# MycroftAI/mycroft-precise

Hardware: NVIDIA H100
Metric: stream-updates/s (16 kHz int16 PCM, 1024-sample chunk -> decoded confidence + trigger) (higher is better)
Workload: dtype f32

## Files before the change

### include/precise_b200.h

```cpp
#ifndef PRECISE_B200_H
#define PRECISE_B200_H

#include <stdint.h>

#ifdef __cplusplus
extern "C" {
#endif

#define PB_ABI_VERSION 2
#define PB_MAX_THRESHOLDS 8
#define PB_MAX_MODELS 8

typedef enum pb_status {
    PB_OK = 0,
    PB_ERR_INVALID = -1,
    PB_ERR_UNSUPPORTED = -2,
    PB_ERR_CUDA = -3,
    PB_ERR_STATE = -4,
    PB_ERR_EOF = -5
} pb_status;

enum { PB_VEC_MELS = 1, PB_VEC_MFCCS = 2, PB_VEC_SPEECHPY_MFCCS = 3  };
enum { PB_ACT_LINEAR = 0, PB_ACT_TANH = 1 };
enum { PB_RACT_HARD_SIGMOID = 0, PB_RACT_SIGMOID = 1 };
// ... 207 lines not shown

int pb_host_alloc(void** out, uint64_t bytes);
int pb_host_free(void* p);

int pb_profile_enable(pb_handle* h, int on);
int pb_profile_reset(pb_handle* h);
int pb_profile_read(pb_handle* h, double ms[4], uint64_t launches[4]);

int pb_get_filterbank(const pb_handle* h, double* h_out);
int64_t pb_get_cdf(const pb_handle* h, double* h_out, int64_t capacity, int32_t* min_out, int32_t* max_out);
int pb_set_cdf(pb_handle* h, const double* h_cd, int64_t len);

int pb_debug_force_generic(pb_handle* h, int on);
int pb_debug_gru_mode(pb_handle* h, int mode);
int pb_debug_k1_mode(pb_handle* h, int mode);
int pb_debug_pool_tiles(pb_handle* h, int warp_only);
int pb_debug_corpus_pool_rows(pb_handle* h, int64_t rows);
int pb_debug_corpus_pool_scan(pb_handle* h, int32_t nm, int32_t groups_fast);
int pb_debug_corpus_pairs_batch(pb_handle* h, int64_t windows);
int pb_debug_tc_dft_power(const int16_t* x512, double* power257);
int pb_debug_mma_dft_power(const int16_t* x512, double* power257);
int pb_debug_tc_mfcc_frame(const pb_config* cfg, const int16_t* x512, float* out);
int pb_debug_tc3_mfcc_frame(const pb_config* cfg, const int16_t* x512, float* out, double* power257);

const char* pb_last_error(void);
int pb_abi_version(void);
const char* pb_build_info(void);

#ifdef __cplusplus
}
// ... 3 lines not shown
```

### mycroft_precise_b200/core.py

```python
import ctypes as C
import os

import numpy as np

from .params import ListenerParams

_HERE = os.path.dirname(os.path.abspath(__file__))
PB_MAX_THRESHOLDS = 8
PB_MAX_MODELS = 8
PB_ABI_VERSION = 2
CORPUS_SCHEDULES = {'listener': 0, 'simulate': 1}
FRONT_END_FIELDS = ('sample_rate', 'window_samples', 'hop_samples', 'n_fft', 'n_filt', 'n_mfcc', 'n_features',
                    'use_delta', 'vectorizer')


class PBError(RuntimeError):
    pass


class pb_config(C.Structure):
    _fields_ = [
        ('abi_version', C.c_int32), ('device', C.c_int32), ('max_streams', C.c_int32),
        ('chunk_samples', C.c_int32),
        ('sample_rate', C.c_int32), ('window_samples', C.c_int32), ('hop_samples', C.c_int32),
# ... 78 lines not shown
    'pb_generate': (C.c_int, [_VP, _VP, _VP, _I64, _VP, _VP, _I64, _VP, _I64, _VP, _I64, _VP, _I64, _I64, _I32, _VP, _VP, _VP]),
    'pb_train_opts_default': (C.c_int, [C.POINTER(pb_train_opts)]),
    'pb_train': (C.c_int, [_VP, _VP, _I64, _VP, _VP, _I64, _VP, _VP, _I64, C.POINTER(pb_train_opts), _VP, _VP, _VP, _VP]),
    'pb_train_loss': (C.c_int, [_VP, _VP, _I64, _VP, _VP, _I64, _VP, _VP, _I64, C.c_float, C.c_float, _I32, _VP, _VP, _VP, _VP]),
    'pb_host_alloc': (C.c_int, [C.POINTER(_VP), C.c_uint64]),
    'pb_host_free': (C.c_int, [_VP]),
    'pb_profile_enable': (C.c_int, [_VP, C.c_int]),
    'pb_profile_reset': (C.c_int, [_VP]),
    'pb_profile_read': (C.c_int, [_VP, C.POINTER(C.c_double), C.POINTER(C.c_uint64)]),
    'pb_get_filterbank': (C.c_int, [_VP, _VP]),
    'pb_get_cdf': (_I64, [_VP, _VP, _I64, C.POINTER(_I32), C.POINTER(_I32)]),
    'pb_set_cdf': (C.c_int, [_VP, _VP, _I64]),
    'pb_debug_force_generic': (C.c_int, [_VP, C.c_int]),
    'pb_debug_gru_mode': (C.c_int, [_VP, C.c_int]),
    'pb_debug_k1_mode': (C.c_int, [_VP, C.c_int]),
    'pb_debug_pool_tiles': (C.c_int, [_VP, C.c_int]),
    'pb_debug_corpus_pool_rows': (C.c_int, [_VP, _I64]),
    'pb_debug_corpus_pool_scan': (C.c_int, [_VP, _I32, _I32]),
    'pb_debug_corpus_pairs_batch': (C.c_int, [_VP, _I64]),
    'pb_debug_tc_dft_power': (C.c_int, [_VP, _VP]),
    'pb_debug_mma_dft_power': (C.c_int, [_VP, _VP]),
    'pb_debug_tc_mfcc_frame': (C.c_int, [_VP, _VP, _VP]),
    'pb_debug_tc3_mfcc_frame': (C.c_int, [_VP, _VP, _VP, _VP]),
    'pb_last_error': (C.c_char_p, []),
    'pb_abi_version': (C.c_int, []),
    'pb_build_info': (C.c_char_p, []),
}

_lib = None

# ... 918 lines not shown
        cnt = C.c_uint64(0)
        vp = _np_ptr
        check(self.lib.pb_update_host(self._h, vp(pcm_np), vp(ids_np), n, vp(raw_np), vp(conf_np), vp(fired_np),
                                      C.cast(C.byref(cnt), C.c_void_p)))
        return int(cnt.value)

    def gru_mode(self, mode):
        check(self.lib.pb_debug_gru_mode(self._h, int(mode)))

    def force_generic(self, on=True):
        check(self.lib.pb_debug_force_generic(self._h, int(on)))

    def k1_mode(self, mode):
        check(self.lib.pb_debug_k1_mode(self._h, int(mode)))

    def profile(self, on=True):
        check(self.lib.pb_profile_enable(self._h, int(on)))
        check(self.lib.pb_profile_reset(self._h))

    def profile_read(self):
        ms = (C.c_double * 4)()
        ln = (C.c_uint64 * 4)()
        check(self.lib.pb_profile_read(self._h, ms, ln))
        return list(ms), list(ln)

    def filterbank(self) -> np.ndarray:
        fb = np.zeros((self.params.n_filt, self.params.n_fft // 2 + 1), dtype=np.float64)
        check(self.lib.pb_get_filterbank(self._h, fb.ctypes.data_as(C.c_void_p)))
        return fb

# ... 22 lines not shown
```

### mycroft_precise_b200/csrc/api.cu

```cuda
#include <cuda_runtime.h>
#include <math.h>
#include <stdarg.h>
#include <stdint.h>
#include <stdio.h>
#include <string.h>

#include <algorithm>
#include <map>
#include <cuda_fp16.h>
#include <limits>
#include <memory>
#include <mutex>
#include <new>
#include <string>
#include <utility>
#include <vector>

#include "../../include/precise_b200.h"
#include "gru_kernels.cuh"
#include "gru_bank.cuh"
#include "gru_wg.cuh"
#include "gru_wide.cuh"
#include "mfcc_kernels.cuh"
#include "mfcc_fast.cuh"
// ... 129 lines not shown
    int mm_parity = 0;
    bool fast_ok = false;
    int npl = 0, maxc = 0, nol = 0;
    DevArray<float4> d_ptab;
    DevArray<unsigned char> d_ctab;
    DevArray<float> d_dct_t;
    bool pipe_fixed = false;
    DevArray<int4> d_pm_off; DevArray<float4> d_pm_w; DevArray<uint4> d_pm_crow; DevArray<float4> d_pm_dct;
    std::vector<double> fb;
    DevArray<float> d_wrise, d_wfall, d_dct;
    DevArray<int> d_grid;
    DevArray<float2> d_tw_stage, d_tw_post, d_tw_any;
    DevArray<long long> d_n_samples;
    DevArray<int16_t> d_tail;
    DevArray<float> d_ring;
    std::vector<Network> models;
    bool routed = false;
    std::vector<uint8_t> route_mask;
    int64_t subs[PB_MAX_MODELS] = {};
    DevArray<uint8_t> d_route;
    DevArray<int2> d_route_list;
    DevArray<unsigned> d_route_count;
    cudaEvent_t route_ev = nullptr;
    bool history = false;
    int64_t hist_samples = 0;
    int hist_cap = 0;
    int hist_rows = 0;
    DevArray<int16_t> d_hist;
    DevArray<int> d_hist_row;
    DevArray<long long> d_hist_start;
// ... 52 lines not shown
    bool pool_warp_only = false;
    bool pool_trig_set = false;
    std::vector<StreamTrig> pool_trig_host;
    DevArray<TrigRec> d_pool_trig_rec;
    cudaStream_t pipe[HOST_PIPE] = {nullptr, nullptr, nullptr};
    cudaEvent_t pipe_ev[HOST_PIPE] = {nullptr, nullptr, nullptr};
    DevArray<int16_t> d_stage_pcm[HOST_PIPE];
    DevArray<int> d_stage_ids[HOST_PIPE];
    DevArray<float> d_stage_raw[HOST_PIPE];
    DevArray<double> d_stage_conf[HOST_PIPE];
    DevArray<uint8_t> d_stage_fired[HOST_PIPE];
    DevArray<unsigned long long> d_count;
    unsigned long long* h_count_pinned = nullptr;
    bool profiling = false;
    ProfSlot prof[N_PROFILE_SLOTS];

    pb_handle() = default;
    pb_handle(const pb_handle&) = delete;
    pb_handle& operator=(const pb_handle&) = delete;
    ~pb_handle() {
        if (h_count_pinned) cudaFreeHost(h_count_pinned);
        for (int i = 0; i < HOST_PIPE; ++i) {
            if (pipe[i]) cudaStreamDestroy(pipe[i]);
            if (pipe_ev[i]) cudaEventDestroy(pipe_ev[i]);
        }
        for (auto& p : prof)
            for (auto e : p.ev) cudaEventDestroy(e);
        if (route_ev) cudaEventDestroy(route_ev);
        if (corpus_ev) cudaEventDestroy(corpus_ev);
        if (pool_ev) cudaEventDestroy(pool_ev);
    }
};

struct MelHost {
    std::vector<int> grid;
    std::vector<float> wrise, wfall;
    std::vector<double> fb;
};

static int build_mel(const pb_config& c, int n_bins, MelHost& mel) {
    const int nb = n_bins, nf = c.n_filt;
    const double top = 1127.0 * log(1.0 + (double)c.sample_rate / 700.0);
    std::vector<int>& grid = mel.grid;
    std::vector<double>& fb = mel.fb;
    grid.assign(nf + 2, 0);
    long long shift = 0, prev = -1;
    if (c.vectorizer == PB_VEC_SPEECHPY_MFCCS) {
// ... 288 lines not shown
        std::vector<float4> pd((size_t)16 * NF / 4, make_float4(0.f, 0.f, 0.f, 0.f));
        for (int k = 0; k < h->n_out; ++k)
            for (int n = 0; n < NF; ++n) reinterpret_cast<float*>(pd.data())[(size_t)k * NF + n] = dct[(size_t)k * NF + n];
        CK(h->d_pm_off.upload(poff));
        CK(h->d_pm_w.upload(pw));
        CK(h->d_pm_crow.upload(crow));
        CK(h->d_pm_dct.upload(pd));
    }
    const size_t S = (size_t)c.max_streams;
    CK(h->d_n_samples.alloc(S));
    CK(h->d_tail.alloc(S * h->tail_cap));
    CK(h->d_ring.alloc(S * h->ring_rows * h->row_stride));
    CK(cudaMemset(h->d_n_samples.get(), 0, S * sizeof(long long)));
    CK(cudaMemset(h->d_tail.get(), 0, S * h->tail_cap * sizeof(int16_t)));
    CK(cudaMemset(h->d_ring.get(), 0, S * h->ring_rows * h->row_stride * sizeof(float)));
    CK(h->d_count.alloc(1));
    CK(cudaMemset(h->d_count.get(), 0, sizeof(unsigned long long)));
    CK(ensure_dyn_smem(mfcc_batch_kernel<int16_t, true>, (size_t)(h->k1_batch_smem)));
    CK(ensure_dyn_smem(mfcc_batch_kernel<int16_t, false>, (size_t)(h->k1_batch_smem)));
    CK(ensure_dyn_smem(mfcc_batch_kernel<float, true>, (size_t)(h->k1_batch_smem)));
    CK(ensure_dyn_smem(mfcc_batch_kernel<float, false>, (size_t)(h->k1_batch_smem)));
    CK(ensure_dyn_smem(mfcc_fast_batch_kernel, (size_t)(h->k1_fast_smem)));
    CK(ensure_dyn_smem(mfcc_fast_stream_kernel<false>, (size_t)(h->k1_fast_smem)));
    CK(ensure_dyn_smem(mfcc_fast_stream_kernel<true>, (size_t)(h->k1_fast_smem)));
    {
        auto kp = h->pipe_fixed ? mfcc_pipe_stream_kernel<K1P_FIX_NPL, K1P_FIX_MAXC, K1P_FIX_NF, K1P_FIX_NOUT> : mfcc_pipe_stream_kernel<0, 0, 0, 0>;
        CK(ensure_dyn_smem(kp, (size_t)(h->k1_pipe_smem)));
        CK(cudaFuncSetAttribute(kp, cudaFuncAttributePreferredSharedMemoryCarveout, (int)cudaSharedmemCarveoutMaxShared));
    }
    CK(ensure_dyn_smem(mfcc_stream_kernel<true>, (size_t)(h->k1_stream_smem)));
    CK(ensure_dyn_smem(mfcc_stream_kernel<false>, (size_t)(h->k1_stream_smem)));
    CK(ensure_dyn_smem(mfcc_stream_kernel<false, true>, (size_t)(h->k1_stream_smem)));
    CK(ensure_dyn_smem(mfcc_ragged_stream_kernel, (size_t)(h->k1_ragged_smem)));
    CK(ensure_dyn_smem(mfcc_fast_corpus_kernel, (size_t)(h->k1_fast_smem)));
    CK(ensure_dyn_smem(mfcc_corpus_kernel, (size_t)(h->k1_batch_smem)));

    Network net;
    net.cfg = c;
    build_cdf(net);
    CK(upload_network_state(net, S));
    h->models.push_back(std::move(net));
// ... 176 lines not shown
        CK(ensure_dyn_smem(gru_tiled_kernel<false>, tiled_smem));
    }
    net.w = std::move(w);
    return PB_OK;
}

PB_API int pb_load_weights(pb_handle* h, const float* kernel, const float* recurrent, const float* bias,
                    const float* dense_w, float dense_b) {
    if (!h || !kernel || !recurrent || !bias || !dense_w) return fail(PB_ERR_INVALID, "null argument");
    CK(cudaSetDevice(h->cfg.device));
    return load_weights(h->models[0], h->feat, kernel, recurrent, bias, dense_w, dense_b);
}

struct ProfScope {
    pb_handle* h; int slot; cudaStream_t s; int idx = -1;
    ProfScope(pb_handle* h_, int slot_, cudaStream_t s_) : h(h_), slot(slot_), s(s_) {
        if (!h->profiling) return;
        ProfSlot& p = h->prof[slot];
        if (p.used + 2 > (int)p.ev.size()) {
            if ((int)p.ev.size() >= 2 * PROFILE_POOL) {
                for (int i = 0; i + 1 < p.used; i += 2) {
                    cudaEventSynchronize(p.ev[i + 1]);
                    float ms = 0; cudaEventElapsedTime(&ms, p.ev[i], p.ev[i + 1]); p.ms += ms;
                }
                p.used = 0;
            } else {
                cudaEvent_t a, b; cudaEventCreate(&a); cudaEventCreate(&b); p.ev.push_back(a); p.ev.push_back(b);
            }
        }
        idx = p.used; p.used += 2; p.launches++;
        cudaEventRecord(p.ev[idx], s);
    }
    ~ProfScope() { if (idx >= 0) cudaEventRecord(h->prof[slot].ev[idx + 1], s); }
};

PB_API int pb_debug_gru_mode(pb_handle* h, int mode) {
    if (!h) return fail(PB_ERR_INVALID, "null handle");
    if (mode < 0 || mode > 2) return fail(PB_ERR_INVALID, "gru mode must be 0 (automatic), 1 (CUDA-core kernel) or 2 (tensor-core kernel)");
    h->models[0].gru_mode = mode;
    return PB_OK;
}

PB_API int pb_debug_k1_mode(pb_handle* h, int mode) {
    if (!h) return fail(PB_ERR_INVALID, "null handle");
    if (mode < 0 || mode > 6 || mode == 1) return fail(PB_ERR_INVALID, "k1 mode must be 0 (automatic), 2 (FFT kernel, lean set-up, not pipelined), 3 (FFT kernel, 64-bit set-up), 4 (tensor-core DFT stage 2), 5 (both DFT stages on the tensor cores) or 6 (5 with a shuffle epilogue)");
    if (mode != 0 && h->ragged) return fail(PB_ERR_STATE, "k1 modes 2-6 need 16-byte-aligned stream state, which a handle loses with its first pb_update_ragged");
    if (mode >= 4 && !h->mma_ok) return fail(PB_ERR_UNSUPPORTED, "the tensor-core MFCC tick needs n_fft = 512 = frame length, hop >= 512 (a multiple of 8), chunk >= hop (a multiple of 8), n_filt <= 32, MFCC vectorizer");
    if ((mode == 2 || mode == 3) && !h->fast_ok) return fail(PB_ERR_UNSUPPORTED, "k1 modes 2 and 3 need the aligned geometry of the fast MFCC kernels");
    h->k1_mode = mode;
    return PB_OK;
}

PB_API int pb_debug_tc_dft_power(const int16_t* x512, double* power257) {
    if (!x512 || !power257) return fail(PB_ERR_INVALID, "null argument");
// ... 65 lines not shown
}

PB_API int pb_debug_mma_dft_power(const int16_t* x512, double* power257) {
    if (!x512 || !power257) return fail(PB_ERR_INVALID, "null argument");
    mm_host_power(x512, power257);
    return PB_OK;
}

PB_API int pb_debug_force_generic(pb_handle* h, int on) { if (!h) return fail(PB_ERR_INVALID, "null handle"); h->force_generic = on != 0; return PB_OK; }

PB_API int pb_profile_enable(pb_handle* h, int on) { if (!h) return fail(PB_ERR_INVALID, "null handle"); h->profiling = on != 0; return PB_OK; }

PB_API int pb_profile_reset(pb_handle* h) {
    if (!h) return fail(PB_ERR_INVALID, "null handle");
    for (auto& p : h->prof) { p.used = 0; p.ms = 0; p.launches = 0; }
    return PB_OK;
}

PB_API int pb_profile_read(pb_handle* h, double ms[4], uint64_t launches[4]) {
    if (!h) return fail(PB_ERR_INVALID, "null handle");
    CK(cudaSetDevice(h->cfg.device));
    for (int s = 0; s < N_PROFILE_SLOTS; ++s) {
        ProfSlot& p = h->prof[s];
        for (int i = 0; i + 1 < p.used; i += 2) {
            CK(cudaEventSynchronize(p.ev[i + 1]));
            float t = 0; CK(cudaEventElapsedTime(&t, p.ev[i], p.ev[i + 1])); p.ms += t;
        }
        p.used = 0;
        if (ms) ms[s] = p.ms;
        if (launches) launches[s] = p.launches;
    }
    return PB_OK;
}

static MelTables mel_tables(const pb_handle* h) {
    MelTables t;
// ... 102 lines not shown
    const NetWeights& nw = *net.w;
    BankModelW& w = P.w[slot];
    w.bfrag = nw.bfrag16.get(); w.xfrag = nw.xfrag16.get(); w.bias = nw.mma_bias.get(); w.wd = nw.mma_wd.get(); w.bd = nw.bd;
    w.act = net.cfg.activation; w.ract = net.cfg.recurrent_activation;
    P.dp[slot] = decode_params(net);
    P.o[slot] = o;
}

template <int NM, bool RING, bool KERAS_ACT>
static int launch_bank_act(const BankParams& P, const K2In& in, int64_t n, cudaStream_t s) {
    constexpr size_t smem = (size_t)NM * BANK_MODEL_SMEM + (bank_stages(NM, RING) ? BANK_STAGE_SMEM : 0);
    const int per_cta = (MMA_THREADS / 32) * 16;
    const int grid = (int)((n + per_cta - 1) / per_cta);
    if constexpr (NM == 1) {
        if constexpr (smem > 48 * 1024) CK(ensure_dyn_smem(gru_wg_kernel<RING, KERAS_ACT>, smem));
        gru_wg_kernel<RING, KERAS_ACT><<<grid, MMA_THREADS, smem, s>>>(P, in, n);
    } else {
        if constexpr (smem > 48 * 1024) CK(ensure_dyn_smem(gru_bank_kernel<NM, RING, KERAS_ACT>, smem));
        gru_bank_kernel<NM, RING, KERAS_ACT><<<grid, MMA_THREADS, smem, s>>>(P, in, n);
    }
    CK(cudaGetLastError());
    return PB_OK;
}

template <int NM, bool RING>
static int launch_bank_nm(const BankParams& P, const K2In& in, int64_t n, cudaStream_t s) {
    if constexpr (NM == 1)
        if (P.w[0].act == PB_ACT_LINEAR && P.w[0].ract == PB_RACT_HARD_SIGMOID) return launch_bank_act<1, RING, true>(P, in, n, s);
    return launch_bank_act<NM, RING, false>(P, in, n, s);
}

// ... 109 lines not shown
    const int grid = (int)std::min<int64_t>((n + K1_STREAMS_PER_CTA - 1) / K1_STREAMS_PER_CTA, (int64_t)h->sm_count * 4);
    ProfScope ps(h, 0, s);
    for (int64_t off = 0; off < max_len; off += rg.sub) {
        rg.round_off = off;
        if (fast)
            mfcc_ragged_stream_kernel<<<gridf, K1F_THREADS, h->k1_ragged_smem, s>>>(d_pcm, rg, d_ids, (int)n, h->cfg.hop_samples, spw, scale,
                                                                                   mel_tables(h), fast_tables(h), st);
        else
            mfcc_stream_kernel<false, true><<<grid, K1_THREADS, h->k1_stream_smem, s>>>(d_pcm, d_ids, (int)n, 0, 0, h->cfg.hop_samples, h->used,
                                                                                       scale, mel_tables(h), st, rg);
        CK(cudaGetLastError());
    }
    return PB_OK;
}

static int launch_stream_mfcc(pb_handle* h, const int16_t* d_pcm, const int32_t* d_ids, int64_t n, cudaStream_t s) {
    if (h->ragged) return launch_ragged_mfcc(h, d_pcm, nullptr, h->cfg.chunk_samples, d_ids, n, s);
    const bool pairs = (h->cfg.chunk_samples % 2 == 0) && (h->cfg.hop_samples % 2 == 0) && (h->used % 2 == 0) &&
                       ((uintptr_t)d_pcm % 4 == 0);
    const int64_t tiles = (n + K1_STREAMS_PER_CTA - 1) / K1_STREAMS_PER_CTA;
    const int grid = (int)std::min<int64_t>(tiles, (int64_t)h->sm_count * 4);
    const float inv = 1.0f / 32768.0f, scale = inv * inv / (float)h->cfg.n_fft;
    const StreamState st = stream_state(h);
    ProfScope ps(h, 0, s);
    if (h->k1_mode >= 4 && h->mma_ok && (uintptr_t)d_pcm % 16 == 0 && !h->force_generic) {
        int rc = ensure_mma_tables(h);
        if (rc != PB_OK) return rc;
        MmTables t;
        t.b1 = h->d_mm_b1.get(); t.b2 = h->d_mm_b2.get(); t.tw = h->d_mm_tw.get();
        t.pscale = inv * inv / (float)h->cfg.n_fft * 1024.f;
        const int par = h->mm_parity;
        h->mm_parity ^= 1;
        MmRec* recs = h->d_mm_recs.get();
        unsigned int* counters = h->d_mm_counters.get();
        mfcc_mma_plan_kernel<<<(int)((n + MM_PLAN_THREADS - 1) / MM_PLAN_THREADS), MM_PLAN_THREADS, 0, s>>>(
            d_pcm, d_ids, (int)n, h->cfg.chunk_samples, h->cfg.hop_samples, st, recs, counters, par);
        const int64_t max_tiles = (n * std::max(1, h->max_new) + MM_FRAMES - 1) / MM_FRAMES;
        const int gm = (int)std::min<int64_t>((max_tiles + MM_WARPS - 1) / MM_WARPS, h->sm_count);
        if (h->k1_mode == 4)
            mfcc_mma_kernel<false, false><<<gm, MM_THREADS, sizeof(MmSmem), s>>>(t, mel_tables(h), recs, counters, par);
        else if (h->k1_mode == 5)
            mfcc_mma_kernel<true, false><<<gm, MM_THREADS, sizeof(MmSmem), s>>>(t, mel_tables(h), recs, counters, par);
        else
            mfcc_mma_kernel<true, true><<<gm, MM_THREADS, sizeof(MmSmem), s>>>(t, mel_tables(h), recs, counters, par);
    } else if (h->fast_ok && h->max_new <= 8 && h->cfg.chunk_samples % 8 == 0 && (uintptr_t)d_pcm % 16 == 0 && !h->force_generic) {
        const int64_t warps_total = (int64_t)h->sm_count * 4 * K1F_WARPS;
        const int spw = (int)std::max<int64_t>(1, std::min<int64_t>(K1F_STREAMS_PER_WARP, (n + warps_total - 1) / warps_total));
        const int64_t tilesf = (n + spw - 1) / spw;
        const int gridf = (int)std::min<int64_t>((tilesf + K1F_WARPS - 1) / K1F_WARPS, (int64_t)h->sm_count * 4);
        if (h->k1_mode == 0) {
            const int gridp = (int)std::min<int64_t>((tilesf + K1F_WARPS - 1) / K1F_WARPS, (int64_t)h->sm_count * K1P_CTAS_PER_SM);
            PipeMelTables pm;
            pm.poff = h->d_pm_off.get(); pm.pw = h->d_pm_w.get(); pm.crow = h->d_pm_crow.get(); pm.dct = h->d_pm_dct.get();
            auto kp = h->pipe_fixed ? mfcc_pipe_stream_kernel<K1P_FIX_NPL, K1P_FIX_MAXC, K1P_FIX_NF, K1P_FIX_NOUT> : mfcc_pipe_stream_kernel<0, 0, 0, 0>;
            kp<<<gridp, K1F_THREADS, h->k1_pipe_smem, s>>>(d_pcm, d_ids, (int)n, h->cfg.chunk_samples, h->cfg.hop_samples, spw, scale,
                                                           mel_tables(h), fast_tables(h), pm, st);
        } else if (h->k1_mode != 3)
            mfcc_fast_stream_kernel<true><<<gridf, K1F_THREADS, h->k1_fast_smem, s>>>(d_pcm, d_ids, (int)n, h->cfg.chunk_samples, h->cfg.hop_samples, spw, scale,
                                                                                      mel_tables(h), fast_tables(h), st);
        else
            mfcc_fast_stream_kernel<false><<<gridf, K1F_THREADS, h->k1_fast_smem, s>>>(d_pcm, d_ids, (int)n, h->cfg.chunk_samples, h->cfg.hop_samples, spw, scale,
                                                                                       mel_tables(h), fast_tables(h), st);
    } else if (h->max_new > 8) {
        const int sub = std::max(1, 6 * h->cfg.hop_samples);
        for (int off = 0; off < h->cfg.chunk_samples; off += sub)
            mfcc_stream_kernel<false><<<grid, K1_THREADS, h->k1_stream_smem, s>>>(d_pcm + off, d_ids, (int)n, std::min(sub, h->cfg.chunk_samples - off),
                                                                                    h->cfg.chunk_samples, h->cfg.hop_samples, h->used, scale, mel_tables(h), st, RaggedIn{});
    } else if (pairs)
        mfcc_stream_kernel<true><<<grid, K1_THREADS, h->k1_stream_smem, s>>>(d_pcm, d_ids, (int)n, h->cfg.chunk_samples, h->cfg.chunk_samples, h->cfg.hop_samples, h->used, scale, mel_tables(h), st, RaggedIn{});
    else
        mfcc_stream_kernel<false><<<grid, K1_THREADS, h->k1_stream_smem, s>>>(d_pcm, d_ids, (int)n, h->cfg.chunk_samples, h->cfg.chunk_samples, h->cfg.hop_samples, h->used, scale, mel_tables(h), st, RaggedIn{});
// ... 11 lines not shown
                          int64_t n, cudaStream_t s) {
    if (!h->history) return PB_OK;
    RaggedIn rg{};
    rg.offsets = reinterpret_cast<const long long*>(d_offsets);
    rg.max_len = max_len;
    rg.chunk = h->cfg.chunk_samples;
    rg.sub = (int)std::min<int64_t>(max_len, INT32_MAX);
    const int per = HIST_THREADS / 32;
    ProfScope ps(h, 3, s);
    history_append_kernel<<<(unsigned)((n + per - 1) / per), HIST_THREADS, 0, s>>>(d_pcm, rg, d_ids, (int)n, h->d_n_samples.get(),
                                                                                  hist_pool(h));
    CK(cudaGetLastError());
    return PB_OK;
}

static int tick_mfcc(pb_handle* h, const int16_t* d_pcm, const int32_t* d_ids, int64_t n, cudaStream_t s) {
    const int rc = append_history(h, d_pcm, nullptr, h->cfg.chunk_samples, d_ids, n, s);
    return rc != PB_OK ? rc : launch_stream_mfcc(h, d_pcm, d_ids, n, s);
}

PB_API int pb_update_vectors(pb_handle* h, const int16_t* d_pcm, const int32_t* d_ids, int64_t n, void* stream) {
    int rc = check_tick(h, d_pcm, n);
    if (rc != PB_OK || n == 0) return rc;
    CK(cudaSetDevice(h->cfg.device));
    return tick_mfcc(h, d_pcm, d_ids, n, (cudaStream_t)stream);
}

static K2In stream_k2in(const pb_handle* h, const int32_t* d_ids) {
    K2In in{};
    in.ring = h->d_ring.get(); in.n_samples = h->d_n_samples.get(); in.ids = d_ids;
    in.ring_rows = h->ring_rows; in.row_stride = h->row_stride; in.window = h->rel_window; in.hop = h->cfg.hop_samples;
    in.T = h->cfg.n_features; in.F_base = h->n_out; in.use_delta = h->cfg.use_delta;
    return in;
}

static int score_model0(pb_handle* h, const int32_t* d_ids, int64_t n, float* d_raw, double* d_conf, uint8_t* d_fired,
                        unsigned long long* d_count, cudaStream_t s) {
    const Network& net = h->models[0];
    K2Out o{};
    o.raw = d_raw; o.conf = d_conf; o.fired = d_fired; o.count = d_count; o.trig = net.trig.get();
    if (!h->routed && !net.trig_set) return launch_gru(h, net, stream_k2in(h, d_ids), true, n, o, s);
    TrigTick t{};
    t.ids = d_ids; t.n = n;
    int nt = 0;
    if (net.trig_set) defer_trigger(t, nt, net, 1u, o);
    ProfScope ps(h, 1, s);
    if (h->routed) {
        RouteOut r{};
        r.raw = d_raw; r.conf = d_conf; r.fired = d_fired; r.M = 1;
        route_kernel<<<(int)((n + 255) / 256), 256, 0, s>>>(h->d_route.get(), d_ids, n, r);
        CK(cudaGetLastError());
        if (h->subs[0] == 0) return PB_OK;
        o.route = h->d_route.get(); o.route_bit = 1;
        t.route = h->d_route.get();
    }
    const int rc = launch_gru_kernels(net, h->feat, stream_k2in(h, d_ids), true, n, o, s);
    return rc != PB_OK ? rc : launch_trigger(t, nt, s);
}

PB_API int pb_update(pb_handle* h, const int16_t* d_pcm, const int32_t* d_ids, int64_t n, float* d_raw, double* d_conf,
              uint8_t* d_fired, unsigned long long* d_count, void* stream) {
    int rc = check_tick(h, d_pcm, n);
    if (rc != PB_OK || n == 0) return rc;
    const Network& net = h->models[0];
    if (!net.w) return fail(PB_ERR_STATE, "pb_load_weights has not been called");
    if (!d_conf) return fail(PB_ERR_INVALID, "null d_conf");
    CK(cudaSetDevice(h->cfg.device));
    cudaStream_t s = (cudaStream_t)stream;
    rc = tick_mfcc(h, d_pcm, d_ids, n, s);
    if (rc != PB_OK) return rc;
    return score_model0(h, d_ids, n, d_raw, d_conf, d_fired, d_count, s);
}


static int check_front_end(const pb_handle* h, const pb_config& c) {
    if (c.abi_version != PB_ABI_VERSION) return fail(PB_ERR_INVALID, "abi_version %d != %d", c.abi_version, PB_ABI_VERSION);
#define PB_SAME_FRONT_END(f)                                                                                  \
    if (c.f != h->cfg.f)                                                                                      \
        return fail(PB_ERR_INVALID, "front-end field %s = %d differs from the handle's %d: the models of a bank share one MFCC front end", \
                    #f, (int)c.f, (int)h->cfg.f)
    PB_SAME_FRONT_END(sample_rate); PB_SAME_FRONT_END(window_samples); PB_SAME_FRONT_END(hop_samples); PB_SAME_FRONT_END(n_fft);
    PB_SAME_FRONT_END(n_filt); PB_SAME_FRONT_END(n_mfcc); PB_SAME_FRONT_END(n_features); PB_SAME_FRONT_END(use_delta);
    PB_SAME_FRONT_END(vectorizer); PB_SAME_FRONT_END(chunk_samples); PB_SAME_FRONT_END(device);
#undef PB_SAME_FRONT_END
    return PB_OK;
}
// ... 2490 lines not shown
```

### mycroft_precise_b200/csrc/gru_kernels.cuh

```cuda
#pragma once
#include <cuda_runtime.h>
#include <stdint.h>

namespace pb {

struct DecodeParams {
    const double* cd;
    int cd_len;
    int min_out, out_range;
    double center;
    double hot_threshold;
    int trigger_level;
    int trigger_reset;
    int legacy_f64;
};

struct K2Out {
    float* raw;
    float* logit;
    double* conf;
    uint8_t* fired;
    unsigned long long* count;
    int* trig;
    const uint8_t* route;
    unsigned route_bit;
};

struct K2In {
    const float* inputs;
    const float* ring;
    union {
        const long long* n_samples;
        const long long* starts;
    };
    const int* ids;
    int ring_rows, row_stride, window, hop;
    int T, F_base;
    int use_delta;
};

__device__ __forceinline__ const float* input_row(const K2In& in, long long i, int t) {
    return in.inputs + ((in.starts ? in.starts[i] : i * in.T) + t) * (long long)in.row_stride;
}

__device__ __forceinline__ float input_value(const K2In& in, long long i, int t, int f) {
    const float* row = input_row(in, i, t);
    if (!in.use_delta || f < in.F_base) return __ldg(row + f);
    const int fb = f - in.F_base;
    return t > 0 ? __ldg(row + fb) - __ldg(row + fb - in.row_stride) : 0.f;
}

__device__ __forceinline__ float hard_sigmoid(float x) { return fminf(fmaxf(fmaf(0.2f, x, 0.5f), 0.f), 1.f); }
__device__ __forceinline__ float sigmoid32(float x) { return 1.f / (1.f + expf(-x)); }
// ... 471 lines not shown
```

### mycroft_precise_b200/csrc/gru_wg.cuh

```cuda
#pragma once
#include <stdint.h>

#include "gru_bank.cuh"

namespace pb {

constexpr int WG_TILE_BYTES = 72 * 16 * 2;
__host__ __device__ constexpr int wg_b_offset(int k, int n) { return (n >> 3) * 256 + (k >> 3) * 128 + (n & 7) * 16 + (k & 7) * 2; }

__device__ __forceinline__ uint64_t wg_desc(const void* p) {
    const uint32_t a = (uint32_t)__cvta_generic_to_shared(p);
    return (uint64_t)((a & 0x3ffff) >> 4) | ((uint64_t)(128 >> 4) << 16) | ((uint64_t)(256 >> 4) << 32);
}

__device__ __forceinline__ void wg_fence() { asm volatile("wgmma.fence.sync.aligned;" ::: "memory"); }
__device__ __forceinline__ void wg_commit() { asm volatile("wgmma.commit_group.sync.aligned;" ::: "memory"); }
template <int N>
__device__ __forceinline__ void wg_wait() { asm volatile("wgmma.wait_group.sync.aligned %0;" :: "n"(N) : "memory"); }
__device__ __forceinline__ void wg_fence_smem() { asm volatile("fence.proxy.async.shared::cta;" ::: "memory"); }
template <int N>
__device__ __forceinline__ void wg_fence_regs(float* d) {
#pragma unroll
    for (int i = 0; i < N; ++i) asm volatile("" : "+f"(d[i]) :: "memory");
}
// ... 22 lines not shown
                 "{%0,%1,%2,%3,%4,%5,%6,%7,%8,%9,%10,%11,%12,%13,%14,%15,%16,%17,%18,%19,%20,%21,%22,%23,"
                 "%24,%25,%26,%27,%28,%29,%30,%31,%32,%33,%34,%35}, {%36,%37,%38,%39}, %40, p, 1, 1, 0;\n}\n"
                 : "+f"(d[0]), "+f"(d[1]), "+f"(d[2]), "+f"(d[3]), "+f"(d[4]), "+f"(d[5]), "+f"(d[6]), "+f"(d[7]),
                   "+f"(d[8]), "+f"(d[9]), "+f"(d[10]), "+f"(d[11]), "+f"(d[12]), "+f"(d[13]), "+f"(d[14]), "+f"(d[15]),
                   "+f"(d[16]), "+f"(d[17]), "+f"(d[18]), "+f"(d[19]), "+f"(d[20]), "+f"(d[21]), "+f"(d[22]), "+f"(d[23]),
                   "+f"(d[24]), "+f"(d[25]), "+f"(d[26]), "+f"(d[27]), "+f"(d[28]), "+f"(d[29]), "+f"(d[30]), "+f"(d[31]),
                   "+f"(d[32]), "+f"(d[33]), "+f"(d[34]), "+f"(d[35])
                 : "r"(a[0]), "r"(a[1]), "r"(a[2]), "r"(a[3]), "l"(desc), "r"(1));
}

template <bool RING, bool KERAS_ACT>
__global__ void __launch_bounds__(MMA_THREADS, 4)
gru_wg_kernel(const __grid_constant__ BankParams P, K2In in, long long n) {
    extern __shared__ __align__(16) unsigned char bank_smem[];
    const BankModelW& w = P.w[0];
    unsigned char* sW = bank_smem;
    float* sb = reinterpret_cast<float*>(bank_smem + BANK_FRAG_U4 * 16);
    for (int e = threadIdx.x; e < 3 * MMA_NT * 32; e += blockDim.x) {
        const int kt = e / (MMA_NT * 32), nt = (e / 32) % MMA_NT, lane = e & 31, col = 8 * nt + (lane >> 2), k = 2 * (lane & 3);
        const uint4 f = kt < 2 ? __ldg(w.bfrag + e) : __ldg(w.xfrag + e - 2 * MMA_NT * 32);
        unsigned char* hi = sW + (kt == 2 ? 0 : 2 + 2 * kt) * WG_TILE_BYTES;
        unsigned char* lo = hi + WG_TILE_BYTES;
        *reinterpret_cast<uint32_t*>(hi + wg_b_offset(k, col)) = f.x;
        *reinterpret_cast<uint32_t*>(hi + wg_b_offset(k + 8, col)) = f.y;
        *reinterpret_cast<uint32_t*>(lo + wg_b_offset(k, col)) = f.z;
        *reinterpret_cast<uint32_t*>(lo + wg_b_offset(k + 8, col)) = f.w;
    }
    for (int e = threadIdx.x; e < 72; e += blockDim.x) sb[e] = __ldg(w.bias + e);
    for (int e = threadIdx.x; e < 24; e += blockDim.x) sb[72 + e] = __ldg(w.wd + e);
    wg_fence_smem();
// ... 6 lines not shown
    int sid[2];
    bool ok[2];
#pragma unroll
    for (int hf = 0; hf < 2; ++hf) {
        idx[hf] = base + g + 8 * hf;
        ok[hf] = idx[hf] < n;
        sid[hf] = RING && ok[hf] ? (in.ids ? in.ids[idx[hf]] : (int)idx[hf]) : 0;
    }
    float* stage = reinterpret_cast<float*>(bank_smem + BANK_MODEL_SMEM) + warp * 2 * BANK_STAGE_BUF;
    const int cs = lane >> 1;
    const bool cok = STAGE && base + cs < n;
    RingCursor cur;
    cur.stride = 0;
    if (cok) {
        const int csid = in.ids ? in.ids[base + cs] : (int)(base + cs);
        const long long ns = in.n_samples[csid];
        cur.init(in, csid, ns >= in.window ? (ns - in.window) / in.hop + 1 : 0);
    }
    if (STAGE) {
        bank_stage(stage, cur, cok, cs, 0, in.T, in.ring, lane);
        cp_async_commit();
        bank_stage(stage + BANK_STAGE_BUF, cur, cok, cs, BANK_STAGE_STEPS, in.T, in.ring, lane);
        cp_async_commit();
    }
    const uint64_t dXh = wg_desc(sW), dXl = wg_desc(sW + WG_TILE_BYTES), dU0h = wg_desc(sW + 2 * WG_TILE_BYTES),
                   dU0l = wg_desc(sW + 3 * WG_TILE_BYTES), dU1h = wg_desc(sW + 4 * WG_TILE_BYTES), dU1l = wg_desc(sW + 5 * WG_TILE_BYTES);
    constexpr uint64_t C6 = (6 * 256) >> 4;
    const int ra = w.ract, ac = w.act;
    int chunk = 0, cr = 0;
    float h[3][4] = {};
// ... 104 lines not shown
    }
    if (STAGE) cp_async_wait<0>();
    const float* sWd = sb + 72;
#pragma unroll
    for (int hf = 0; hf < 2; ++hf) {
        float part = 0.f;
#pragma unroll
        for (int nt = 0; nt < 3; ++nt) {
            part = fmaf(h[nt][2 * hf], sWd[8 * nt + 2 * t], part);
            part = fmaf(h[nt][2 * hf + 1], sWd[8 * nt + 2 * t + 1], part);
        }
        part += __shfl_xor_sync(0xffffffffu, part, 1);
        part += __shfl_xor_sync(0xffffffffu, part, 2);
        epilogue(part + w.bd, t == 0 && ok[hf], idx[hf], sid[hf], P.dp[0], P.o[0]);
    }
}

}
```

### mycroft_precise_b200/csrc/mfcc_fast.cuh

```cuda
#pragma once
#include <cuda_runtime.h>
#include <stdint.h>
#include "fft512.cuh"
#include "mfcc_kernels.cuh"

namespace pb {

__device__ __forceinline__ uint32_t smem_u32(const void* p) { return (uint32_t)__cvta_generic_to_shared(p); }

__device__ __forceinline__ void mbar_init(unsigned long long* bar, uint32_t count) {
    asm volatile("mbarrier.init.shared::cta.b64 [%0], %1;" ::"r"(smem_u32(bar)), "r"(count) : "memory");
}
__device__ __forceinline__ void mbar_arrive(unsigned long long* bar) {
    asm volatile("mbarrier.arrive.shared::cta.b64 _, [%0];" ::"r"(smem_u32(bar)) : "memory");
}
__device__ __forceinline__ void mbar_expect_tx(unsigned long long* bar, uint32_t bytes) {
    asm volatile("mbarrier.arrive.expect_tx.shared::cta.b64 _, [%0], %1;" ::"r"(smem_u32(bar)), "r"(bytes) : "memory");
}
__device__ __forceinline__ void bulk_g2s(void* dst, const void* src, uint32_t bytes, unsigned long long* bar) {
    asm volatile("cp.async.bulk.shared::cluster.global.mbarrier::complete_tx::bytes [%0], [%1], %2, [%3];"
                 ::"r"(smem_u32(dst)), "l"(src), "r"(bytes), "r"(smem_u32(bar)) : "memory");
}
__device__ __forceinline__ void mbar_wait(unsigned long long* bar, uint32_t parity) {
    uint32_t ok;
// ... 445 lines not shown
    fft512_power(z, lc, P, P, scale, l16, active);
    float* part = reinterpret_cast<float*>(ws.in[stage][half]);
    if (l16 == 0) { P[K1F_ZERO_BIN] = 0.f; part[128] = 0.f; }
    if constexpr (NPL == 0) {
        int eoff[8];
#pragma unroll
        for (int i = 0; i < 8; ++i) eoff[i] = ((i + rot) & 7) * 16 + l16;
        __syncwarp();
        mel16<K1P_MEL_UQ, K1P_MEL_UC>(P, tb, ft, t, part, part + K1F_PART, eoff, l16, active, out);
    } else {
        __syncwarp();
        mel16_fixed<NPL, MAXC, NF, NOUT>(P, pt, part, part + K1F_PART, lane, l16, active, out);
    }
}

template <int NPL, int MAXC, int NF, int NOUT>
__global__ void __launch_bounds__(K1F_THREADS, K1P_CTAS_PER_SM)
mfcc_pipe_stream_kernel(const int16_t* __restrict__ pcm, const int* __restrict__ ids, int n, int chunk, int hop, int spw,
                        float scale, MelTables tab, FastTables ft, PipeMelTables pmt, StreamState st) {
    extern __shared__ __align__(16) unsigned char smem_raw[];
    K1PWarp* wsm = reinterpret_cast<K1PWarp*>(smem_raw);
    const int lane = threadIdx.x & 31, warp = threadIdx.x >> 5, l16 = lane & 15, half = lane >> 4;
    K1PWarp& ws = wsm[warp];
    float2* tws = reinterpret_cast<float2*>(smem_raw + K1F_WARPS * sizeof(K1PWarp));
    K1FTab tb{};
    PipeMelTables pt{};
    if constexpr (NPL == 0) {
        tb = load_fast_tables(reinterpret_cast<unsigned char*>(tws + 256), tab, ft);
    } else {
        constexpr int NO = NPL * 2 * 32, NW = NPL * 4 * 32, NC = PipeMelShape<NPL, NF>::ROWS, ND = 16 * NF / 4;
        int4* po = reinterpret_cast<int4*>(tws + 256);
        float4* pw = reinterpret_cast<float4*>(po + NO);
        uint4* pc = reinterpret_cast<uint4*>(pw + NW);
        float4* pd = reinterpret_cast<float4*>(pc + NC);
        for (int k = threadIdx.x; k < NO; k += blockDim.x) po[k] = __ldg(pmt.poff + k);
        for (int k = threadIdx.x; k < NW; k += blockDim.x) pw[k] = __ldg(pmt.pw + k);
        for (int k = threadIdx.x; k < NC; k += blockDim.x) pc[k] = __ldg(pmt.crow + k);
// ... 129 lines not shown
                    int t = 0;
#pragma unroll
                    for (int b = 8; b >= 1; b >>= 1)
                        if (t + b < spw && ws.st_vbeg[t + b] <= e) t += b;
                    const int vi = e - ws.st_vbeg[t];
                    const int cn = ws.st_cnt[t];
                    v[u] = __ldg(reinterpret_cast<const int4*>(pcm + (long long)(base + t) * chunk + ws.st_ts0[t]) + vi);
                    dst[u] = reinterpret_cast<int4*>(st.tail + (long long)ws.st_id[t] * st.tail_cap + (cn >> 16)) + vi;
                }
            }
#pragma unroll
            for (int u = 0; u < K1P_TAIL_INFLIGHT; ++u)
                if (dst[u] != nullptr) *dst[u] = v[u];
        }
        __syncwarp();
        sid = sid_next;
        n0 = n0_next;
    }
}

}
```

Before: 336.5 million.

## Overlap MFCC and GRU kernels with programmatic launch and per-stream ready flags

Adds a tick-overlap path in which the pipelined MFCC kernel triggers programmatic dependent launch early and publishes a per-stream epoch flag with release semantics once each stream's features are written. The GRU workgroup kernel is launched with programmatic stream serialization and spins with acquire loads on each stream's flag before reading its ring. This is meant to hide the kernel boundary and launch gap between feature extraction and scoring. It costs spin-waiting that occupies SM resources, an epoch counter that must be reset on wraparound, and some device-timer span bookkeeping when profiling.

```diff
diff --git a/include/precise_b200.h b/include/precise_b200.h
--- a/include/precise_b200.h
+++ b/include/precise_b200.h
@@ -245,6 +245,9 @@
 int pb_debug_force_generic(pb_handle* h, int on);
 int pb_debug_gru_mode(pb_handle* h, int mode);
 int pb_debug_k1_mode(pb_handle* h, int mode);
+int pb_debug_tick_overlap(pb_handle* h, int on);
+int pb_debug_tick_epoch(pb_handle* h, uint32_t epoch);
+int64_t pb_debug_tick_overlaps(const pb_handle* h);
 int pb_debug_pool_tiles(pb_handle* h, int warp_only);
 int pb_debug_corpus_pool_rows(pb_handle* h, int64_t rows);
 int pb_debug_corpus_pool_scan(pb_handle* h, int32_t nm, int32_t groups_fast);
diff --git a/mycroft_precise_b200/core.py b/mycroft_precise_b200/core.py
--- a/mycroft_precise_b200/core.py
+++ b/mycroft_precise_b200/core.py
@@ -116,6 +116,9 @@
     'pb_debug_force_generic': (C.c_int, [_VP, C.c_int]),
     'pb_debug_gru_mode': (C.c_int, [_VP, C.c_int]),
     'pb_debug_k1_mode': (C.c_int, [_VP, C.c_int]),
+    'pb_debug_tick_overlap': (C.c_int, [_VP, C.c_int]),
+    'pb_debug_tick_epoch': (C.c_int, [_VP, C.c_uint32]),
+    'pb_debug_tick_overlaps': (C.c_int64, [_VP]),
     'pb_debug_pool_tiles': (C.c_int, [_VP, C.c_int]),
     'pb_debug_corpus_pool_rows': (C.c_int, [_VP, _I64]),
     'pb_debug_corpus_pool_scan': (C.c_int, [_VP, _I32, _I32]),
@@ -1064,6 +1067,15 @@
     def k1_mode(self, mode):
         check(self.lib.pb_debug_k1_mode(self._h, int(mode)))
 
+    def tick_overlap(self, on=True):
+        check(self.lib.pb_debug_tick_overlap(self._h, int(on)))
+
+    def tick_epoch(self, epoch):
+        check(self.lib.pb_debug_tick_epoch(self._h, int(epoch)))
+
+    def tick_overlaps(self):
+        return int(self.lib.pb_debug_tick_overlaps(self._h))
+
     def profile(self, on=True):
         check(self.lib.pb_profile_enable(self._h, int(on)))
         check(self.lib.pb_profile_reset(self._h))
diff --git a/mycroft_precise_b200/csrc/api.cu b/mycroft_precise_b200/csrc/api.cu
--- a/mycroft_precise_b200/csrc/api.cu
+++ b/mycroft_precise_b200/csrc/api.cu
@@ -167,6 +167,10 @@
     DevArray<long long> d_n_samples;
     DevArray<int16_t> d_tail;
     DevArray<float> d_ring;
+    bool tick_overlap = true;
+    DevArray<unsigned> d_ready;
+    unsigned tick_epoch = 0;
+    int64_t tick_overlaps = 0;
     std::vector<Network> models;
     bool routed = false;
     std::vector<uint8_t> route_mask;
@@ -249,6 +253,8 @@
     unsigned long long* h_count_pinned = nullptr;
     bool profiling = false;
     ProfSlot prof[N_PROFILE_SLOTS];
+    DevArray<unsigned long long> d_span;
+    int span_used = 0;
 
     pb_handle() = default;
     pb_handle(const pb_handle&) = delete;
@@ -266,6 +272,14 @@
         if (pool_ev) cudaEventDestroy(pool_ev);
     }
 };
+
+using PipeKernel = void (*)(const int16_t*, const int*, int, int, int, int, float, MelTables, FastTables, PipeMelTables, StreamState,
+                            TickSync);
+template <bool SYNC>
+static PipeKernel pipe_kernel(bool pipe_fixed) {
+    if (pipe_fixed) return mfcc_pipe_stream_kernel<K1P_FIX_NPL, K1P_FIX_MAXC, K1P_FIX_NF, K1P_FIX_NOUT, SYNC>;
+    return mfcc_pipe_stream_kernel<0, 0, 0, 0, SYNC>;
+}
 
 struct MelHost {
     std::vector<int> grid;
@@ -584,6 +598,8 @@
     CK(cudaMemset(h->d_n_samples.get(), 0, S * sizeof(long long)));
     CK(cudaMemset(h->d_tail.get(), 0, S * h->tail_cap * sizeof(int16_t)));
     CK(cudaMemset(h->d_ring.get(), 0, S * h->ring_rows * h->row_stride * sizeof(float)));
+    CK(h->d_ready.alloc(S));
+    CK(cudaMemset(h->d_ready.get(), 0, S * sizeof(unsigned)));
     CK(h->d_count.alloc(1));
     CK(cudaMemset(h->d_count.get(), 0, sizeof(unsigned long long)));
     CK(ensure_dyn_smem(mfcc_batch_kernel<int16_t, true>, (size_t)(h->k1_batch_smem)));
@@ -593,8 +609,7 @@
     CK(ensure_dyn_smem(mfcc_fast_batch_kernel, (size_t)(h->k1_fast_smem)));
     CK(ensure_dyn_smem(mfcc_fast_stream_kernel<false>, (size_t)(h->k1_fast_smem)));
     CK(ensure_dyn_smem(mfcc_fast_stream_kernel<true>, (size_t)(h->k1_fast_smem)));
-    {
-        auto kp = h->pipe_fixed ? mfcc_pipe_stream_kernel<K1P_FIX_NPL, K1P_FIX_MAXC, K1P_FIX_NF, K1P_FIX_NOUT> : mfcc_pipe_stream_kernel<0, 0, 0, 0>;
+    for (PipeKernel kp : {pipe_kernel<false>(h->pipe_fixed), pipe_kernel<true>(h->pipe_fixed)}) {
         CK(ensure_dyn_smem(kp, (size_t)(h->k1_pipe_smem)));
         CK(cudaFuncSetAttribute(kp, cudaFuncAttributePreferredSharedMemoryCarveout, (int)cudaSharedmemCarveoutMaxShared));
     }
@@ -801,8 +816,8 @@
 
 struct ProfScope {
     pb_handle* h; int slot; cudaStream_t s; int idx = -1;
-    ProfScope(pb_handle* h_, int slot_, cudaStream_t s_) : h(h_), slot(slot_), s(s_) {
-        if (!h->profiling) return;
+    ProfScope(pb_handle* h_, int slot_, cudaStream_t s_, bool on = true) : h(h_), slot(slot_), s(s_) {
+        if (!h->profiling || !on) return;
         ProfSlot& p = h->prof[slot];
         if (p.used + 2 > (int)p.ev.size()) {
             if ((int)p.ev.size() >= 2 * PROFILE_POOL) {
@@ -825,6 +840,20 @@
     if (!h) return fail(PB_ERR_INVALID, "null handle");
     if (mode < 0 || mode > 2) return fail(PB_ERR_INVALID, "gru mode must be 0 (automatic), 1 (CUDA-core kernel) or 2 (tensor-core kernel)");
     h->models[0].gru_mode = mode;
+    return PB_OK;
+}
+
+PB_API int pb_debug_tick_overlap(pb_handle* h, int on) {
+    if (!h) return fail(PB_ERR_INVALID, "null handle");
+    h->tick_overlap = on != 0;
+    return PB_OK;
+}
+
+PB_API int64_t pb_debug_tick_overlaps(const pb_handle* h) { return h ? h->tick_overlaps : -1; }
+
+PB_API int pb_debug_tick_epoch(pb_handle* h, uint32_t epoch) {
+    if (!h) return fail(PB_ERR_INVALID, "null handle");
+    h->tick_epoch = epoch;
     return PB_OK;
 }
 
@@ -920,12 +949,29 @@
 PB_API int pb_profile_reset(pb_handle* h) {
     if (!h) return fail(PB_ERR_INVALID, "null handle");
     for (auto& p : h->prof) { p.used = 0; p.ms = 0; p.launches = 0; }
+    h->span_used = 0;
+    return PB_OK;
+}
+
+static int fold_spans(pb_handle* h) {
+    if (h->span_used == 0) return PB_OK;
+    std::vector<unsigned long long> r((size_t)4 * h->span_used);
+    CK(cudaDeviceSynchronize());
+    CK(cudaMemcpy(r.data(), h->d_span.get(), r.size() * sizeof(unsigned long long), cudaMemcpyDeviceToHost));
+    for (int i = 0; i < h->span_used; ++i) {
+        const unsigned long long* x = &r[(size_t)4 * i];
+        h->prof[0].ms += (double)(x[1] - ~x[0]) * 1e-6;
+        h->prof[1].ms += (double)(x[3] - ~x[2]) * 1e-6;
+    }
+    h->span_used = 0;
     return PB_OK;
 }
 
 PB_API int pb_profile_read(pb_handle* h, double ms[4], uint64_t launches[4]) {
     if (!h) return fail(PB_ERR_INVALID, "null handle");
     CK(cudaSetDevice(h->cfg.device));
+    const int rc = fold_spans(h);
+    if (rc != PB_OK) return rc;
     for (int s = 0; s < N_PROFILE_SLOTS; ++s) {
         ProfSlot& p = h->prof[s];
         for (int i = 0; i + 1 < p.used; i += 2) {
@@ -1058,7 +1104,19 @@
     const int grid = (int)((n + per_cta - 1) / per_cta);
     if constexpr (NM == 1) {
         if constexpr (smem > 48 * 1024) CK(ensure_dyn_smem(gru_wg_kernel<RING, KERAS_ACT>, smem));
-        gru_wg_kernel<RING, KERAS_ACT><<<grid, MMA_THREADS, smem, s>>>(P, in, n);
+        if (RING && in.sync.ready != nullptr) {
+            cudaLaunchConfig_t cfg = {};
+            cfg.gridDim = dim3(grid); cfg.blockDim = dim3(MMA_THREADS); cfg.dynamicSmemBytes = smem; cfg.stream = s;
+            cudaLaunchAttribute at[2];
+            at[0].id = cudaLaunchAttributeProgrammaticStreamSerialization;
+            at[0].val.programmaticStreamSerializationAllowed = 1;
+            at[1].id = cudaLaunchAttributePreferredSharedMemoryCarveout;
+            at[1].val.sharedMemCarveout = (unsigned)cudaSharedmemCarveoutMaxShared;
+            cfg.attrs = at; cfg.numAttrs = 2;
+            CK(cudaLaunchKernelEx(&cfg, gru_wg_kernel<RING, KERAS_ACT>, P, in, (long long)n));
+        } else {
+            gru_wg_kernel<RING, KERAS_ACT><<<grid, MMA_THREADS, smem, s>>>(P, in, n);
+        }
     } else {
         if constexpr (smem > 48 * 1024) CK(ensure_dyn_smem(gru_bank_kernel<NM, RING, KERAS_ACT>, smem));
         gru_bank_kernel<NM, RING, KERAS_ACT><<<grid, MMA_THREADS, smem, s>>>(P, in, n);
@@ -1198,7 +1256,38 @@
     return PB_OK;
 }
 
-static int launch_stream_mfcc(pb_handle* h, const int16_t* d_pcm, const int32_t* d_ids, int64_t n, cudaStream_t s) {
+static int next_tick_epoch(pb_handle* h, unsigned& epoch) {
+    if (++h->tick_epoch == 0) {
+        CK(cudaDeviceSynchronize());
+        CK(cudaMemset(h->d_ready.get(), 0, (size_t)h->cfg.max_streams * sizeof(unsigned)));
+        CK(cudaDeviceSynchronize());
+        h->tick_epoch = 1;
+    }
+    epoch = h->tick_epoch;
+    return PB_OK;
+}
+
+static int launch_stream_mfcc(pb_handle* h, const int16_t* d_pcm, const int32_t* d_ids, int64_t n, cudaStream_t s,
+                              TickSync* sync = nullptr) {
+    const bool fast = !h->ragged && h->fast_ok && h->max_new <= 8 && h->cfg.chunk_samples % 8 == 0 && (uintptr_t)d_pcm % 16 == 0 &&
+                      !h->force_generic;
+    if (sync != nullptr && !(fast && h->k1_mode == 0)) *sync = TickSync{};
+    const bool overlap = sync != nullptr && sync->ready != nullptr;
+    if (overlap) {
+        int rc = next_tick_epoch(h, sync->epoch);
+        if (rc != PB_OK) return rc;
+        sync->span = nullptr;
+        if (h->profiling) {
+            if (h->span_used == PROFILE_POOL) {
+                rc = fold_spans(h);
+                if (rc != PB_OK) return rc;
+            }
+            if (!h->d_span.get()) CK(h->d_span.alloc((size_t)4 * PROFILE_POOL));
+            sync->span = h->d_span.get() + (size_t)4 * h->span_used++;
+            CK(cudaMemsetAsync(sync->span, 0, 4 * sizeof(unsigned long long), s));
+            h->prof[0].launches++;
+        }
+    }
     if (h->ragged) return launch_ragged_mfcc(h, d_pcm, nullptr, h->cfg.chunk_samples, d_ids, n, s);
     const bool pairs = (h->cfg.chunk_samples % 2 == 0) && (h->cfg.hop_samples % 2 == 0) && (h->used % 2 == 0) &&
                        ((uintptr_t)d_pcm % 4 == 0);
@@ -1206,7 +1295,7 @@
     const int grid = (int)std::min<int64_t>(tiles, (int64_t)h->sm_count * 4);
     const float inv = 1.0f / 32768.0f, scale = inv * inv / (float)h->cfg.n_fft;
     const StreamState st = stream_state(h);
-    ProfScope ps(h, 0, s);
+    ProfScope ps(h, 0, s, !overlap);
     if (h->k1_mode >= 4 && h->mma_ok && (uintptr_t)d_pcm % 16 == 0 && !h->force_generic) {
         int rc = ensure_mma_tables(h);
         if (rc != PB_OK) return rc;
@@ -1227,7 +1316,7 @@
             mfcc_mma_kernel<true, false><<<gm, MM_THREADS, sizeof(MmSmem), s>>>(t, mel_tables(h), recs, counters, par);
         else
             mfcc_mma_kernel<true, true><<<gm, MM_THREADS, sizeof(MmSmem), s>>>(t, mel_tables(h), recs, counters, par);
-    } else if (h->fast_ok && h->max_new <= 8 && h->cfg.chunk_samples % 8 == 0 && (uintptr_t)d_pcm % 16 == 0 && !h->force_generic) {
+    } else if (fast) {
         const int64_t warps_total = (int64_t)h->sm_count * 4 * K1F_WARPS;
         const int spw = (int)std::max<int64_t>(1, std::min<int64_t>(K1F_STREAMS_PER_WARP, (n + warps_total - 1) / warps_total));
         const int64_t tilesf = (n + spw - 1) / spw;
@@ -1236,9 +1325,9 @@
             const int gridp = (int)std::min<int64_t>((tilesf + K1F_WARPS - 1) / K1F_WARPS, (int64_t)h->sm_count * K1P_CTAS_PER_SM);
             PipeMelTables pm;
             pm.poff = h->d_pm_off.get(); pm.pw = h->d_pm_w.get(); pm.crow = h->d_pm_crow.get(); pm.dct = h->d_pm_dct.get();
-            auto kp = h->pipe_fixed ? mfcc_pipe_stream_kernel<K1P_FIX_NPL, K1P_FIX_MAXC, K1P_FIX_NF, K1P_FIX_NOUT> : mfcc_pipe_stream_kernel<0, 0, 0, 0>;
+            auto kp = overlap ? pipe_kernel<true>(h->pipe_fixed) : pipe_kernel<false>(h->pipe_fixed);
             kp<<<gridp, K1F_THREADS, h->k1_pipe_smem, s>>>(d_pcm, d_ids, (int)n, h->cfg.chunk_samples, h->cfg.hop_samples, spw, scale,
-                                                           mel_tables(h), fast_tables(h), pm, st);
+                                                           mel_tables(h), fast_tables(h), pm, st, overlap ? *sync : TickSync{});
         } else if (h->k1_mode != 3)
             mfcc_fast_stream_kernel<true><<<gridf, K1F_THREADS, h->k1_fast_smem, s>>>(d_pcm, d_ids, (int)n, h->cfg.chunk_samples, h->cfg.hop_samples, spw, scale,
                                                                                       mel_tables(h), fast_tables(h), st);
@@ -1280,9 +1369,9 @@
     return PB_OK;
 }
 
-static int tick_mfcc(pb_handle* h, const int16_t* d_pcm, const int32_t* d_ids, int64_t n, cudaStream_t s) {
+static int tick_mfcc(pb_handle* h, const int16_t* d_pcm, const int32_t* d_ids, int64_t n, cudaStream_t s, TickSync* sync = nullptr) {
     const int rc = append_history(h, d_pcm, nullptr, h->cfg.chunk_samples, d_ids, n, s);
-    return rc != PB_OK ? rc : launch_stream_mfcc(h, d_pcm, d_ids, n, s);
+    return rc != PB_OK ? rc : launch_stream_mfcc(h, d_pcm, d_ids, n, s, sync);
 }
 
 PB_API int pb_update_vectors(pb_handle* h, const int16_t* d_pcm, const int32_t* d_ids, int64_t n, void* stream) {
@@ -1301,11 +1390,18 @@
 }
 
 static int score_model0(pb_handle* h, const int32_t* d_ids, int64_t n, float* d_raw, double* d_conf, uint8_t* d_fired,
-                        unsigned long long* d_count, cudaStream_t s) {
+                        unsigned long long* d_count, cudaStream_t s, const TickSync* sync = nullptr) {
     const Network& net = h->models[0];
     K2Out o{};
     o.raw = d_raw; o.conf = d_conf; o.fired = d_fired; o.count = d_count; o.trig = net.trig.get();
-    if (!h->routed && !net.trig_set) return launch_gru(h, net, stream_k2in(h, d_ids), true, n, o, s);
+    if (!h->routed && !net.trig_set) {
+        K2In in = stream_k2in(h, d_ids);
+        if (sync == nullptr || sync->ready == nullptr) return launch_gru(h, net, in, true, n, o, s);
+        in.sync = *sync;
+        if (h->profiling) h->prof[1].launches++;
+        h->tick_overlaps++;
+        return launch_gru_kernels(net, h->feat, in, true, n, o, s);
+    }
     TrigTick t{};
     t.ids = d_ids; t.n = n;
     int nt = 0;
@@ -1333,9 +1429,13 @@
     if (!d_conf) return fail(PB_ERR_INVALID, "null d_conf");
     CK(cudaSetDevice(h->cfg.device));
     cudaStream_t s = (cudaStream_t)stream;
-    rc = tick_mfcc(h, d_pcm, d_ids, n, s);
-    if (rc != PB_OK) return rc;
-    return score_model0(h, d_ids, n, d_raw, d_conf, d_fired, d_count, s);
+    TickSync sync{};
+    if (h->tick_overlap && !h->routed && !net.trig_set && net.w->small_path && net.gru_mode != 1 &&
+        !(n <= K2_WARP_PATH_MAX && net.gru_mode == 0))
+        sync.ready = h->d_ready.get();
+    rc = tick_mfcc(h, d_pcm, d_ids, n, s, &sync);
+    if (rc != PB_OK) return rc;
+    return score_model0(h, d_ids, n, d_raw, d_conf, d_fired, d_count, s, &sync);
 }
 
 
diff --git a/mycroft_precise_b200/csrc/gru_kernels.cuh b/mycroft_precise_b200/csrc/gru_kernels.cuh
--- a/mycroft_precise_b200/csrc/gru_kernels.cuh
+++ b/mycroft_precise_b200/csrc/gru_kernels.cuh
@@ -1,6 +1,8 @@
 #pragma once
 #include <cuda_runtime.h>
 #include <stdint.h>
+
+#include "tick_sync.cuh"
 
 namespace pb {
 
@@ -37,6 +39,7 @@
     int ring_rows, row_stride, window, hop;
     int T, F_base;
     int use_delta;
+    TickSync sync;
 };
 
 __device__ __forceinline__ const float* input_row(const K2In& in, long long i, int t) {
diff --git a/mycroft_precise_b200/csrc/gru_wg.cuh b/mycroft_precise_b200/csrc/gru_wg.cuh
--- a/mycroft_precise_b200/csrc/gru_wg.cuh
+++ b/mycroft_precise_b200/csrc/gru_wg.cuh
@@ -60,6 +60,7 @@
 gru_wg_kernel(const __grid_constant__ BankParams P, K2In in, long long n) {
     extern __shared__ __align__(16) unsigned char bank_smem[];
     const BankModelW& w = P.w[0];
+    if (RING && threadIdx.x == 0 && in.sync.span != nullptr) span_start(in.sync.span + 2);
     unsigned char* sW = bank_smem;
     float* sb = reinterpret_cast<float*>(bank_smem + BANK_FRAG_U4 * 16);
     for (int e = threadIdx.x; e < 3 * MMA_NT * 32; e += blockDim.x) {
@@ -96,6 +97,7 @@
     cur.stride = 0;
     if (cok) {
         const int csid = in.ids ? in.ids[base + cs] : (int)(base + cs);
+        if (in.sync.ready != nullptr) wait_ready(in.sync.ready, csid, in.sync.epoch);
         const long long ns = in.n_samples[csid];
         cur.init(in, csid, ns >= in.window ? (ns - in.window) / in.hop + 1 : 0);
     }
@@ -230,6 +232,7 @@
         part += __shfl_xor_sync(0xffffffffu, part, 2);
         epilogue(part + w.bd, t == 0 && ok[hf], idx[hf], sid[hf], P.dp[0], P.o[0]);
     }
-}
-
-}
+    if (RING && lane == 0 && in.sync.span != nullptr) span_end(in.sync.span + 2);
+}
+
+}
diff --git a/mycroft_precise_b200/csrc/mfcc_fast.cuh b/mycroft_precise_b200/csrc/mfcc_fast.cuh
--- a/mycroft_precise_b200/csrc/mfcc_fast.cuh
+++ b/mycroft_precise_b200/csrc/mfcc_fast.cuh
@@ -3,6 +3,7 @@
 #include <stdint.h>
 #include "fft512.cuh"
 #include "mfcc_kernels.cuh"
+#include "tick_sync.cuh"
 
 namespace pb {
 
@@ -483,13 +484,15 @@
     }
 }
 
-template <int NPL, int MAXC, int NF, int NOUT>
+template <int NPL, int MAXC, int NF, int NOUT, bool SYNC>
 __global__ void __launch_bounds__(K1F_THREADS, K1P_CTAS_PER_SM)
 mfcc_pipe_stream_kernel(const int16_t* __restrict__ pcm, const int* __restrict__ ids, int n, int chunk, int hop, int spw,
-                        float scale, MelTables tab, FastTables ft, PipeMelTables pmt, StreamState st) {
+                        float scale, MelTables tab, FastTables ft, PipeMelTables pmt, StreamState st, TickSync sync) {
+    if (SYNC) asm volatile("griddepcontrol.launch_dependents;" ::: "memory");
     extern __shared__ __align__(16) unsigned char smem_raw[];
     K1PWarp* wsm = reinterpret_cast<K1PWarp*>(smem_raw);
     const int lane = threadIdx.x & 31, warp = threadIdx.x >> 5, l16 = lane & 15, half = lane >> 4;
+    if (SYNC && threadIdx.x == 0) span_start(sync.span);
     K1PWarp& ws = wsm[warp];
     float2* tws = reinterpret_cast<float2*>(smem_raw + K1F_WARPS * sizeof(K1PWarp));
     K1FTab tb{};
@@ -649,9 +652,14 @@
                 if (dst[u] != nullptr) *dst[u] = v[u];
         }
         __syncwarp();
+        if (SYNC) {
+            __threadfence();
+            if (lane < spw && ws.st_id[lane] >= 0) st_release_gpu(sync.ready + ws.st_id[lane], sync.epoch);
+        }
         sid = sid_next;
         n0 = n0_next;
     }
-}
-
-}
+    if (SYNC && lane == 0) span_end(sync.span);
+}
+
+}
diff --git a/mycroft_precise_b200/csrc/tick_sync.cuh b/mycroft_precise_b200/csrc/tick_sync.cuh
--- /dev/null
+++ b/mycroft_precise_b200/csrc/tick_sync.cuh
@@ -0,0 +1,40 @@
+#pragma once
+#include <stdint.h>
+
+namespace pb {
+
+struct TickSync {
+    unsigned* ready;
+    unsigned epoch;
+    unsigned long long* span;
+};
+
+__device__ __forceinline__ unsigned ld_acquire_gpu(const unsigned* p) {
+    unsigned v;
+    asm volatile("ld.acquire.gpu.global.u32 %0, [%1];" : "=r"(v) : "l"(p) : "memory");
+    return v;
+}
+__device__ __forceinline__ void st_release_gpu(unsigned* p, unsigned v) {
+    asm volatile("st.release.gpu.global.u32 [%0], %1;" :: "l"(p), "r"(v) : "memory");
+}
+__device__ __forceinline__ unsigned long long globaltimer_ns() {
+    unsigned long long t;
+    asm volatile("mov.u64 %0, %%globaltimer;" : "=l"(t));
+    return t;
+}
+__device__ __forceinline__ void span_start(unsigned long long* span) {
+    if (span != nullptr) atomicMax(span, ~globaltimer_ns());
+}
+__device__ __forceinline__ void span_end(unsigned long long* span) {
+    if (span != nullptr) atomicMax(span + 1, globaltimer_ns());
+}
+
+__device__ __forceinline__ void wait_ready(const unsigned* ready, int sid, unsigned epoch) {
+    unsigned ns = 32;
+    while (ld_acquire_gpu(ready + sid) != epoch) {
+        __nanosleep(ns);
+        ns = ns < 512 ? 2 * ns : 512;
+    }
+}
+
+}
```

After: 351.7 million, median of 6. 4.5% higher.
